# BarisYazici/deep-rl-grasping

Measured on NVIDIA H100. Metric: SAC grad-steps/sec (batch 256, 64x64 depth), higher is better.
Workload: dtype bf16x3 (fp32-faithful split, f32 accumulate)

## Files before the change

### deep-rl-grasping_b200/csrc/engine_v2.cu

```cuda
#include <cuda_bf16.h>

#include <algorithm>
#include <cstdio>
#include <cstdlib>
#include <cstring>

#include "sac_internal.cuh"

namespace b2g {
namespace {

struct Gather2Args {
  GatherArgs g;
  uint16_t* s1[2][3];
  uint16_t* fp[3][3];
  int KF;
};

__device__ __forceinline__ void split3(float y, uint16_t& p0, uint16_t& p1, uint16_t& p2) {
  const __nv_bfloat16 h0 = __float2bfloat16_rn(y);
  const float r1 = y - __bfloat162float(h0);
  const __nv_bfloat16 h1 = __float2bfloat16_rn(r1);
  const float r2 = r1 - __bfloat162float(h1);
  p0 = __bfloat16_as_ushort(h0); p1 = __bfloat16_as_ushort(h1); p2 = __bfloat16_as_ushort(__float2bfloat16_rn(r2));
}

template <int Ci>
__device__ __forceinline__ void s2d_half_block(const Gather2Args& a, const unsigned char* __restrict__ src, int it, int which, size_t b) {
  constexpr int CP = s2d_channels(Ci);
  const GatherArgs& g = a.g;
  const int npx = g.H * g.W * Ci;
  const int h = it & 1, X = (it >> 1) & 15, Y = it >> 5;
  const double clip_obs = g.normc[1];
  const bool norm_obs = g.normc[3] != 0.0;
  const float scale = g.scale;
#pragma unroll
  for (int rr = 0; rr < 2; ++rr) {
    const int e0 = ((4 * Y + 2 * h + rr) * g.W + 4 * X) * Ci;
    float y[4 * Ci];
#pragma unroll
    for (int q = 0; q < Ci; ++q) {
      const int e = e0 + 4 * q;
      const float4 v = frame_load4(src, g.fmt, npx, Ci, e);
      float t[4] = {v.x, v.y, v.z, v.w};
      if (norm_obs) {
        const double2 m0 = *reinterpret_cast<const double2*>(g.mean + e), m1 = *reinterpret_cast<const double2*>(g.mean + e + 2);
        const double2 i0 = *reinterpret_cast<const double2*>(g.var + e), i1 = *reinterpret_cast<const double2*>(g.var + e + 2);
        t[0] = (float)fmin(fmax(((double)t[0] - m0.x) * i0.x, -clip_obs), clip_obs);
        t[1] = (float)fmin(fmax(((double)t[1] - m0.y) * i0.y, -clip_obs), clip_obs);
        t[2] = (float)fmin(fmax(((double)t[2] - m1.x) * i1.x, -clip_obs), clip_obs);
        t[3] = (float)fmin(fmax(((double)t[3] - m1.y) * i1.y, -clip_obs), clip_obs);
      }
#pragma unroll
      for (int j = 0; j < 4; ++j) y[4 * q + j] = t[j];
    }
    uint32_t p[3][2 * CP];
#pragma unroll
    for (int k = 0; k < 4 * CP; k += 2) {
      uint16_t q[3][2];
#pragma unroll
      for (int u = 0; u < 2; ++u) {
        const int c = (k + u) / CP, ci = (k + u) % CP;
        if (ci < Ci) split3(y[c * Ci + ci] / scale, q[0][u], q[1][u], q[2][u]);
        else q[0][u] = q[1][u] = q[2][u] = 0;
      }
#pragma unroll
      for (int pl = 0; pl < 3; ++pl) p[pl][k / 2] = (uint32_t)q[pl][0] | ((uint32_t)q[pl][1] << 16);
    }
    const size_t o = b * 4096 * CP + (size_t)((Y * 16 + X) * 16 + 4 * (2 * h + rr)) * CP;
#pragma unroll
    for (int pl = 0; pl < 3; ++pl) {
      if constexpr (CP == 1) {
        *reinterpret_cast<uint2*>(a.s1[which][pl] + o) = make_uint2(p[pl][0], p[pl][1]);
      } else {
        uint4* d = reinterpret_cast<uint4*>(a.s1[which][pl] + o);
        d[0] = make_uint4(p[pl][0], p[pl][1], p[pl][2], p[pl][3]);
        d[1] = make_uint4(p[pl][4], p[pl][5], p[pl][6], p[pl][7]);
      }
    }
  }
}

template <int Ci>
__global__ void __launch_bounds__(512) gather2_kernel(Gather2Args a) {
  const GatherArgs& g = a.g;
  const int b = blockIdx.x, which = blockIdx.y, tid = threadIdx.x;
  const int HW = g.H * g.W, npx = HW * Ci;
  const int Ec = npx + 4;
  long long slot = b;
  if (g.indices) slot = g.indices[b];
  else if (g.rng_counters) {
    slot = philox_slot(g.seed, (unsigned long long)g.rng_counters[4], b, (unsigned long long)g.rng_counters[5]);
    if (g.ring_cap > 0) slot = ring_slot(g.rng_counters[6], (int)slot, g.ring_cap);
    if (g.indices_out && which == 0 && tid == 0) g.indices_out[b] = (int)slot;
  }
  const unsigned char* __restrict__ src =
      g.obs_frame ? g.frames + (size_t)(which ? g.next_frame : g.obs_frame)[slot] * g.frame_bytes
                  : reinterpret_cast<const unsigned char*>((which ? g.next_obs : g.obs) + (size_t)slot * Ec);
  const double clip_obs = g.normc[1];
  const bool norm_obs = g.normc[3] != 0.0;
  const float scale = g.scale;
  for (int it = tid; it < 512; it += blockDim.x) s2d_half_block<Ci>(a, src, it, which, b);
  if (tid == 0 && g.feat_col >= 0) {
    float yy = frame_elem(src, g.fmt, npx, Ci, npx);
    if (norm_obs) yy = (float)fmin(fmax(((double)yy - g.mean[npx]) * g.var[npx], -clip_obs), clip_obs);
    yy = yy / scale;
    uint16_t p0, p1, p2;
    split3(yy, p0, p1, p2);
    const size_t fo = (size_t)b * g.FS + g.feat_col, po = (size_t)b * a.KF + g.feat_col;
    if (which) { g.F_t[fo] = yy; a.fp[2][0][po] = p0; a.fp[2][1][po] = p1; a.fp[2][2][po] = p2; }
    else {
      g.F_pi[fo] = yy; g.F_v[fo] = yy;
      a.fp[0][0][po] = p0; a.fp[0][1][po] = p1; a.fp[0][2][po] = p2;
      a.fp[1][0][po] = p0; a.fp[1][1][po] = p1; a.fp[1][2][po] = p2;
    }
  }
  if (which == 0 && g.act) {
    const int feat_dim = g.act_col;
    if (tid < g.n_act) {
      const float av = g.act[slot * g.n_act + tid];
      g.F_v[(size_t)b * g.FS + feat_dim + tid] = av;
      uint16_t p0, p1, p2;
      split3(av, p0, p1, p2);
      const size_t po = (size_t)b * a.KF + feat_dim + tid;
      a.fp[1][0][po] = p0; a.fp[1][1][po] = p1; a.fp[1][2][po] = p2;
    }
    if (tid == 32) {
      float r = g.rew[slot];
      if (g.normc[4] != 0.0) r = (float)fmin(fmax((double)r * g.normc[0], -g.normc[2]), g.normc[2]);
      g.rew_out[b] = r;
      g.done_out[b] = g.done[slot];
    }
  }
}

struct Plane2Job {
  const float* src;
  uint16_t* dst[3];
  int R, N, np;
  int transpose;
  int ld, off0;
  int k1_ci;
  int tile_start;
};

constexpr int P2_SUB = 4;
__global__ void __launch_bounds__(256) planes2_kernel(const Plane2Job* __restrict__ jobs, const int* __restrict__ cta_job, int cta0) {
  __shared__ float tile[P2_SUB][64][33];
  const int cta = cta0 + blockIdx.x;
  const Plane2Job job = jobs[cta_job[cta]];
  const int t = cta - job.tile_start;
  const int strips_n = (job.N + 32 * P2_SUB - 1) / (32 * P2_SUB);
  const int r0 = (t / strips_n) * 64, nb = (t % strips_n) * 32 * P2_SUB;
  const int tid = threadIdx.x;
  const bool vec_ok = (job.N & 3) == 0;
  float4 v[P2_SUB][2];
#pragma unroll
  for (int q = 0; q < P2_SUB; ++q)
#pragma unroll
    for (int j = 0; j < 2; ++j) {
      const int i = tid + 256 * j, r = r0 + (i >> 3), n = nb + 32 * q + 4 * (i & 7);
      v[q][j] = make_float4(0.f, 0.f, 0.f, 0.f);
      if (r < job.R && n < job.N) {
        const float* sp = job.src + (size_t)r * job.N + n;
        if (vec_ok && n + 3 < job.N) v[q][j] = *reinterpret_cast<const float4*>(sp);
        else { v[q][j].x = sp[0]; if (n + 1 < job.N) v[q][j].y = sp[1]; if (n + 2 < job.N) v[q][j].z = sp[2]; if (n + 3 < job.N) v[q][j].w = sp[3]; }
      }
    }
#pragma unroll
  for (int q = 0; q < P2_SUB; ++q)
#pragma unroll
    for (int j = 0; j < 2; ++j) {
      const int i = tid + 256 * j, rr = i >> 3, c4 = i & 7, r = r0 + rr, n = nb + 32 * q + 4 * c4;
      if (job.transpose) {
        tile[q][rr][4 * c4] = v[q][j].x; tile[q][rr][4 * c4 + 1] = v[q][j].y; tile[q][rr][4 * c4 + 2] = v[q][j].z; tile[q][rr][4 * c4 + 3] = v[q][j].w;
      } else if (r < job.R && n < job.N) {
        const float x[4] = {v[q][j].x, v[q][j].y, v[q][j].z, v[q][j].w};
        uint16_t p[3][4];
#pragma unroll
        for (int u = 0; u < 4; ++u) split3(x[u], p[0][u], p[1][u], p[2][u]);
#pragma unroll
        for (int k = 0; k < 3; ++k) {
          if (k == job.np) break;
          uint16_t* d = job.dst[k] + (size_t)r * job.ld + job.off0 + n;
          if (n + 3 < job.N && (((size_t)r * job.ld + job.off0 + n) & 3) == 0)
            *reinterpret_cast<uint2*>(d) = make_uint2((uint32_t)p[k][0] | ((uint32_t)p[k][1] << 16), (uint32_t)p[k][2] | ((uint32_t)p[k][3] << 16));
          else
            for (int u = 0; u < 4; ++u) if (n + u < job.N) d[u] = p[k][u];
        }
      }
    }
  if (!job.transpose) return;
  __syncthreads();
  const int nn = tid >> 3, g8 = tid & 7, rb = r0 + 8 * g8;
#pragma unroll
  for (int q = 0; q < P2_SUB; ++q) {
    const int n = nb + 32 * q + nn;
    if (n < job.N && rb < job.R) {
      uint16_t p[3][8];
#pragma unroll
      for (int u = 0; u < 8; ++u) split3(tile[q][8 * g8 + u][nn], p[0][u], p[1][u], p[2][u]);
      const size_t o = (size_t)(n + job.off0) * job.ld + rb;
#pragma unroll
      for (int k = 0; k < 3; ++k) {
        if (k == job.np) break;
        uint16_t* d = job.dst[k] + o;
        if (job.k1_ci) {
          for (int u = 0; u < 8; ++u) if (rb + u < job.R) d[conv1_krow(rb + u, job.k1_ci) - rb] = p[k][u];
        } else if (rb + 7 < job.R && (o & 7) == 0)
          *reinterpret_cast<uint4*>(d) = make_uint4((uint32_t)p[k][0] | ((uint32_t)p[k][1] << 16), (uint32_t)p[k][2] | ((uint32_t)p[k][3] << 16),
                                                    (uint32_t)p[k][4] | ((uint32_t)p[k][5] << 16), (uint32_t)p[k][6] | ((uint32_t)p[k][7] << 16));
        else
          for (int u = 0; u < 8; ++u) if (rb + u < job.R) d[u] = p[k][u];
      }
    }
  }
}

int add_maps(V2State& v, uint16_t* const* planes, int np, int rank, std::initializer_list<uint64_t> dims, std::initializer_list<uint64_t> strides_b,
             std::initializer_list<uint32_t> box, std::initializer_list<uint32_t> estr = {}, bool allow_whole = true, int swizzle = 128) {
  uint64_t d[5] = {1, 1, 1, 1, 1}, s[5] = {0, 0, 0, 0, 0};
  uint32_t bx[5] = {1, 1, 1, 1, 1}, es[5] = {1, 1, 1, 1, 1};
  int i = 0; for (auto x : dims) d[i++] = x;
  i = 0; for (auto x : strides_b) s[i++] = x;
  i = 0; for (auto x : box) bx[i++] = x;
  i = 0; for (auto x : estr) es[i++] = x;
  if (rank >= 5 || np < 1) return -1;
  size_t rows = 1;
  for (int k = 1; k < rank; ++k) rows *= (bx[k] + es[k] - 1) / es[k];
  const size_t box_bytes = rows * bx[0] * 2;
  const bool whole = allow_whole && np > 1 && box_bytes % 1024 == 0;
  const long long pitch = np > 1 ? (long long)((const char*)planes[1] - (const char*)planes[0]) : 16;
  for (int p = 2; p < np; ++p)
    if ((const char*)planes[p] - (const char*)planes[p - 1] != pitch) return -1;
  if (pitch <= 0 || pitch % 16) return -1;
  d[rank] = (uint64_t)np; s[rank - 1] = (uint64_t)pitch; bx[rank] = whole ? (uint32_t)np : 1u; es[rank] = 1;
  CUtensorMap m;
  if (cg_encode_map(&m, planes[0], rank + 1, d, s, bx, es, swizzle) != 0) return -1;
  v.maps.push_back(m);
  v.map_whole.push_back(whole ? 1 : 0);
  v.map_box_bytes.push_back((int)box_bytes);
  return (int)v.maps.size() - 1;
}

const V2State* g_mk_state = nullptr;
CgLoad mk_load(int map, int rank, int smem_off) {
  CgLoad L;
  memset(&L, 0, sizeof(L));
  L.map = map; L.rank = rank + 1; L.smem_off = smem_off;
  L.plane_box = g_mk_state->map_whole[map];
  L.box_bytes = g_mk_state->map_box_bytes[map];
  return L;
}

CgProblem kmajor(int planes, int n_tile, int chunks, int n2, int a_box_rows) {
  CgProblem P;
  memset(&P, 0, sizeof(P));
  P.tiles_m = P.tiles_n = P.splits = 1;
  P.chunks = chunks; P.n2 = n2;
  P.planes = planes;
  P.a_off = 0; P.a_pstride = 128 * 128;
  P.b_off = planes * P.a_pstride; P.b_pstride = n_tile * 128;
  P.tx_bytes = planes * (a_box_rows * 128 + n_tile * 128);
  P.mn_major = 0; P.ksteps = 4; P.a_kstep = P.b_kstep = 32; P.a_kstep2 = 64;
  P.a_desc = P.b_desc = cg_desc_bits(128, false, 0); P.a_moff = 64 * 128;
  P.umma_n = n_tile;
  P.nprod = planes == 3 ? 6 : (planes == 2 ? 3 : 1);
  P.d0 = 1 << 20; P.d1 = 1;
  P.grp_stride = 32; P.f_grp = 32; P.bias_grp = 32;
  P.scale = 1.f;
  return P;
}

CgProblem mnmajor(int planes, int kr, int a_atoms, int b_atoms, int chunks) {
  CgProblem P;
  memset(&P, 0, sizeof(P));
  P.tiles_m = P.tiles_n = P.splits = 1;
  P.chunks = chunks; P.n2 = chunks > 0 ? chunks : 1;
  P.planes = planes;
  const int atom = kr * 128;
  P.a_off = 0; P.a_pstride = atom;
  P.b_off = 2 * planes * atom; P.b_pstride = b_atoms * atom;
  P.tx_bytes = planes * (a_atoms + b_atoms) * atom;
  P.mn_major = 1; P.ksteps = kr / 16; P.a_kstep = P.b_kstep = 2048; P.a_kstep2 = 4096;
  P.a_lbo = planes * atom; P.b_lbo = atom;
  P.a_desc = cg_desc_bits(128, true, P.a_lbo); P.b_desc = cg_desc_bits(128, true, P.b_lbo); P.a_moff = P.a_lbo;
  P.umma_n = 64 * b_atoms;
  P.nprod = planes == 3 ? 6 : (planes == 2 ? 3 : 1);
  P.d0 = 1 << 20; P.d1 = 1;
  P.grp_stride = 32; P.f_grp = 32; P.bias_grp = 32;
  P.scale = 1.f;
  P.epi = CG_EPI_WGRAD; P.rows_tile = 128;
  return P;
}

int push_group(b2g_sac* h, std::vector<CgGroup>& list, CgGroup& g, const char* name) {
  g.name = name;
  if (cg_finalize(g, cg_smem_limit()) != 0) return b2g_fail(B2G_EINVAL, std::string("engine v2: stage ring of group ") + name + " does not fit shared memory");
  for (int i = 0; i < g.n; ++i) {
    const CgProblem& P = g.host[i];
    if (P.planes * P.umma_n > 256) return b2g_fail(B2G_EINVAL, std::string("engine v2: planes x tile width exceeds one accumulator buffer (group ") + name + ")");
    if (!cg_shape_supported(P.umma_n, P.nprod, P.mn_major != 0, P.ksteps))
      return b2g_fail(B2G_EINVAL, std::string("engine v2: no cg_kernel instance for the tile shape of a problem in group ") + name);
    if (P.tm_sub > 1 && !cg_epi_handoff(P.epi))
      return b2g_fail(B2G_EINVAL, std::string("engine v2: a banded problem must have an ACT or DGRAD epilogue (group ") + name + ")");
    g.flops += 2.0 * P.tiles_m * 128.0 * P.tiles_n * P.umma_n * P.chunks * 64.0;
  }
  list.push_back(g);
  return 0;
}

struct Wire { int cons, ci, prod, pi, dep_rows, dep_rows_tile, by_chunk; };
int fuse_groups(b2g_sac* h, const std::vector<const CgGroup*>& parts, const std::vector<Wire>& wires, const char* name, std::vector<CgGroup>& out, int& n_ctr) {
  CgGroup f;
  std::vector<int> first(parts.size());
  for (size_t gi = 0; gi < parts.size(); ++gi) {
    first[gi] = f.n;
    for (int i = 0; i < parts[gi]->n; ++i) {
      if (f.n >= CG_MAX_PROBLEMS) return b2g_fail(B2G_EINVAL, std::string("engine v2: too many problems in fused launch ") + name);
      f.host[f.n++] = parts[gi]->host[i];
    }
  }
  std::vector<int> ctr_of(f.n, -1);
  for (const Wire& w : wires) {
    const int pi = first[w.prod] + w.pi, qi = first[w.cons] + w.ci;
    CgProblem& Pp = f.host[pi];
    CgProblem& Pc = f.host[qi];
    if (!cg_epi_handoff(Pp.epi))
      return b2g_fail(B2G_EINVAL, std::string("engine v2: a wired producer must have an ACT or DGRAD epilogue (fused launch ") + name + ")");
    if (Pc.dep_ctr && ctr_of[pi] < 0) {
      ctr_of[pi] = (int)(intptr_t)Pc.dep_ctr - 1;
      Pc.dep_expect += Pp.ws ? Pp.tiles_n : Pp.tiles_n * Pp.splits;
      continue;
    }
    if (Pp.splits > 1 && (Pp.splits - 1) * ((Pp.chunks + Pp.splits - 1) / Pp.splits) >= Pp.chunks)
      return b2g_fail(B2G_EINVAL, std::string("engine v2: a wired split-K producer has an empty split (fused launch ") + name + ")");
    if (ctr_of[pi] < 0) { ctr_of[pi] = n_ctr; n_ctr += Pp.tiles_m; }
    Pc.dep_rows = w.dep_rows; Pc.dep_rows_tile = w.dep_rows_tile; Pc.dep_tiles = Pp.tiles_m; Pc.dep_by_chunk = w.by_chunk;
    Pc.dep_expect = Pp.ws ? Pp.tiles_n : Pp.tiles_n * Pp.splits;
    Pc.dep_ctr = (const int*)(intptr_t)(ctr_of[pi] + 1);
  }
  for (int i = 0; i < f.n; ++i) f.host[i].done_ctr = (int*)(intptr_t)(ctr_of[i] + 1);
  return push_group(h, out, f, name);
}

void bind_counters(std::vector<CgGroup>& groups, int* base) {
  for (CgGroup& g : groups)
    for (int i = 0; i < g.n; ++i) {
      CgProblem& P = g.host[i];
      const intptr_t d = (intptr_t)P.done_ctr, c = (intptr_t)P.dep_ctr;
      P.done_ctr = d ? base + (d - 1) : nullptr;
      P.dep_ctr = c ? base + (c - 1) : nullptr;
    }
}

int check_split(const char* var, int chunks, int splits) {
  auto empty = [chunks](int s) { return (s - 1) * ((chunks + s - 1) / s) >= chunks; };
  if (!empty(splits)) return 0;
  std::string ok;
  for (int s = 1; s <= chunks; ++s)
    if (!empty(s)) ok += (ok.empty() ? "" : ", ") + std::to_string(s);
  return b2g_fail(B2G_EINVAL, std::string(var) + "=" + std::to_string(splits) + " leaves a K-split of " + std::to_string(chunks) +
                                  " chunks empty; use one of " + ok);
}

}

int v2_alloc(b2g_sac* h) {
  V2State& v = h->v2;
  const int B = h->B, Cp = s2d_channels(h->Cimg), K1 = 64 * Cp, KF = v.KF;
  const size_t n1 = (size_t)B * 225 * 32, n2 = (size_t)B * 36 * 64, n3 = (size_t)B * 1024, ns = (size_t)B * 4096 * Cp, nf = (size_t)B * KF;
  uint16_t *bH1, *bH2, *bH3, *bF, *bS;
  if (int rc = dev_alloc(h->allocs, h->stream, &bH1, 9 * n1)) return rc;
  if (int rc = dev_alloc(h->allocs, h->stream, &bH2, 9 * n2)) return rc;
  if (int rc = dev_alloc(h->allocs, h->stream, &bH3, 9 * n3)) return rc;
  if (int rc = dev_alloc(h->allocs, h->stream, &bF, 9 * nf)) return rc;
  if (int rc = dev_alloc(h->allocs, h->stream, &bS, 6 * ns)) return rc;
  for (int n = 0; n < 3; ++n)
    for (int p = 0; p < 3; ++p) {
      v.H1[n][p] = bH1 + (n * 3 + p) * n1; v.H2[n][p] = bH2 + (n * 3 + p) * n2; v.H3[n][p] = bH3 + (n * 3 + p) * n3;
      v.F[n][p] = bF + (n * 3 + p) * nf;
    }
  for (int w = 0; w < 2; ++w) for (int p = 0; p < 3; ++p) v.S[w][p] = bS + (w * 3 + p) * ns;
  if (int rc = dev_alloc(h->allocs, h->stream, &v.z0v, (size_t)B * 3 * h->H)) return rc;
  auto palloc = [&](uint16_t** arr, int np, size_t count) -> int {
    const size_t pitch = (count + 63) / 64 * 64;
    uint16_t* base = nullptr;
    if (int rc = dev_alloc(h->allocs, h->stream, &base, pitch * np)) return rc;
    for (int p = 0; p < np; ++p) arr[p] = base + p * pitch;
    return 0;
  };
  if (int rc = palloc(v.dz0pi, 2, (size_t)B * h->H)) return rc;
  if (int rc = palloc(v.dz0v, 2, (size_t)B * 3 * h->H)) return rc;
  if (int rc = palloc(v.dZ1, 2, (size_t)B * 225 * 64)) return rc;
  for (int n = 0; n < 2; ++n) {
    if (int rc = palloc(v.dZ4[n], 2, (size_t)B * 512)) return rc;
    if (int rc = palloc(v.dZ3[n], 2, n3)) return rc;
    if (int rc = palloc(v.dZ2[n], 2, n2)) return rc;
    if (int rc = palloc(v.W2n[n], 2, 512 * 64)) return rc;
    if (int rc = palloc(v.W3n[n], 2, 576 * 64)) return rc;
    if (int rc = palloc(v.Wfn[n], 2, 1024 * 512)) return rc;
    if (int rc = palloc(v.K0n[n], 2, (size_t)KF * (n == 1 ? 3 : 1) * h->H)) return rc;
  }
  if (int rc = palloc(v.W1T[0], 3, (size_t)64 * K1)) return rc;
  if (int rc = palloc(v.W1T[1], 3, (size_t)32 * K1)) return rc;
  for (int n = 0; n < 3; ++n) {
    if (int rc = palloc(v.W2T[n], 3, 64 * 512)) return rc;
    if (int rc = palloc(v.W3T[n], 3, 64 * 576)) return rc;
    if (int rc = palloc(v.WfT[n], 3, 512 * 1024)) return rc;
    if (int rc = palloc(v.K0T[n], 3, (size_t)(n == 1 ? 3 : 1) * h->H * KF)) return rc;
  }
  return 0;
}

int v2_create(b2g_sac* h) {
  V2State& v = h->v2;
  g_mk_state = &v;
  const int B = h->B, Ci = h->Cimg, Cp = s2d_channels(Ci), K1 = 64 * Cp, KF = v.KF, FS = h->FS, H = h->H;
  const size_t n1 = (size_t)B * 225 * 32;
  const char* nets[3] = {"model/pi", "model/values_fn", "target/values_fn"};
  std::vector<Plane2Job> jobs;
  int start = 0;
  auto add_job = [&](const float* src, int R, int N, uint16_t* const* dst, int np, int transpose, int ld, int off0) {
    Plane2Job j{};
    j.src = src; j.R = R; j.N = N; j.np = np; j.transpose = transpose; j.ld = ld; j.off0 = off0; j.tile_start = start;
    for (int k = 0; k < np; ++k) j.dst[k] = dst[k];
    start += ((R + 63) / 64) * ((N + 32 * P2_SUB - 1) / (32 * P2_SUB));
    jobs.push_back(j);
  };
  add_job(h->p(h->cnn_t("model/pi", 0, "w")), 64 * Ci, 32, v.W1T[0], 3, 1, K1, 0);
  jobs.back().k1_ci = Ci;
  add_job(h->p(h->cnn_t("model/values_fn", 0, "w")), 64 * Ci, 32, v.W1T[0], 3, 1, K1, 32);
  jobs.back().k1_ci = Ci;
  add_job(h->p(h->cnn_t("target/values_fn", 0, "w")), 64 * Ci, 32, v.W1T[1], 3, 1, K1, 0);
  jobs.back().k1_ci = Ci;
  for (int n = 0; n < 3; ++n) {
    add_job(h->p(h->cnn_t(nets[n], 1, "w")), 512, 64, v.W2T[n], 3, 1, 512, 0);
    add_job(h->p(h->cnn_t(nets[n], 2, "w")), 576, 64, v.W3T[n], 3, 1, 576, 0);
    add_job(h->p(h->cnn_t(nets[n], 3, "w")), 1024, 512, v.WfT[n], 3, 1, 1024, 0);
  }
  add_job(h->p("model/pi/fc0/kernel"), h->feat_dim, H, v.K0T[0], 3, 1, KF, 0);
  add_job(h->p("model/values_fn/vf/fc0/kernel"), h->feat_dim, H, v.K0T[1], 3, 1, KF, 0);
  add_job(h->p("model/values_fn/qf1/fc0/kernel"), h->feat_dim + h->A, H, v.K0T[1], 3, 1, KF, H);
  add_job(h->p("model/values_fn/qf2/fc0/kernel"), h->feat_dim + h->A, H, v.K0T[1], 3, 1, KF, 2 * H);
  add_job(h->p("target/values_fn/vf/fc0/kernel"), h->feat_dim, H, v.K0T[2], 3, 1, KF, 0);
  v.plane_ctas_fwd = start;
  for (int n = 0; n < 2; ++n) {
    add_job(h->p(h->cnn_t(nets[n], 1, "w")), 512, 64, v.W2n[n], 2, 0, 64, 0);
    add_job(h->p(h->cnn_t(nets[n], 2, "w")), 576, 64, v.W3n[n], 2, 0, 64, 0);
    add_job(h->p(h->cnn_t(nets[n], 3, "w")), 1024, 512, v.Wfn[n], 2, 0, 512, 0);
  }
  add_job(h->p("model/pi/fc0/kernel"), h->feat_dim, H, v.K0n[0], 2, 0, H, 0);
  add_job(h->p("model/values_fn/vf/fc0/kernel"), h->feat_dim, H, v.K0n[1], 2, 0, 3 * H, 0);
  add_job(h->p("model/values_fn/qf1/fc0/kernel"), h->feat_dim + h->A, H, v.K0n[1], 2, 0, 3 * H, H);
  add_job(h->p("model/values_fn/qf2/fc0/kernel"), h->feat_dim + h->A, H, v.K0n[1], 2, 0, 3 * H, 2 * H);
  v.n_plane_jobs = (int)jobs.size();
  v.plane_ctas = start;
  Plane2Job* dj = nullptr;
  if (int rc = dev_alloc(h->allocs, h->stream, &dj, jobs.size())) return rc;
  CK(cudaMemcpyAsync(dj, jobs.data(), jobs.size() * sizeof(Plane2Job), cudaMemcpyHostToDevice, h->stream));
  CK(cudaStreamSynchronize(h->stream));
  v.plane_jobs = dj;
  {
    std::vector<int> cj((size_t)start);
    for (size_t k = 0; k < jobs.size(); ++k)
      for (int t = jobs[k].tile_start; t < (k + 1 < jobs.size() ? jobs[k + 1].tile_start : start); ++t) cj[t] = (int)k;
    if (int rc = upload_table(h->allocs, h->stream, cj, &v.plane_cta_job)) return rc;
  }

  { const char* e = getenv("B2G_SPLIT_FC1"); v.split_fc1 = e ? std::max(1, atoi(e)) : 3; }
  { const char* e = getenv("B2G_SPLIT_FC1_DGRAD"); v.split_fc1_dgrad = e ? std::max(1, atoi(e)) : 1; }
  const int NP = 3;
  const long long h1_net = (long long)3 * n1;
  {
    CgGroup g;
    for (int w = 0; w < 2; ++w) {
      const int N = w == 0 ? 64 : 32;
      const int mA = Cp == 1 ? add_maps(v, v.S[w], NP, 3, {32, 15, (uint64_t)B * 16}, {32, 512}, {32, 16, 8}, {}, true, 64)
                             : add_maps(v, v.S[w], NP, 3, {64, 16, (uint64_t)B * 16}, {128, 2048}, {64, 16, 8});
      const int mB = add_maps(v, v.W1T[w], NP, 2, {(uint64_t)K1, (uint64_t)N}, {(uint64_t)K1 * 2}, {64, (uint32_t)N});
      if (mA < 0 || mB < 0) return b2g_fail(B2G_ECUDA, "engine v2: cuTensorMapEncodeTiled failed (conv1)");
      CgProblem P;
      if (Cp == 1) {
        P = kmajor(NP, N, 1, 1, 128);
        P.a_pstride = 128 * 64; P.a_kstep = 32; P.a_kstep2 = NP * P.a_pstride;
        P.b_off = 2 * P.a_kstep2;
        P.tx_bytes = NP * (2 * 128 * 64 + N * 128);
        P.a_desc = cg_desc_bits(64, false, 0); P.a_moff = 64 * 64;
        P.nloads = 3;
        for (int a = 0; a < 2; ++a) { P.ld[a] = mk_load(mA, 3, a * P.a_kstep2); P.ld[a].c0[2] = a; P.ld[a].d_tm[2] = 8; }
        P.ld[2] = mk_load(mB, 2, P.b_off);
      } else {
        P = kmajor(NP, N, 4, 2, 128);
        P.nloads = 2;
        P.ld[0] = mk_load(mA, 3, 0); P.ld[0].d_tm[2] = 8; P.ld[0].d_c1[2] = 1; P.ld[0].d_c2[1] = 1;
        P.ld[1] = mk_load(mB, 2, P.b_off); P.ld[1].d_c1[0] = 128; P.ld[1].d_c2[0] = 64;
      }
      P.tiles_m = 2 * B;
      P.epi = CG_EPI_ACT; P.rows_tile = 128; P.lim_rows = 2 * B * 128;
      P.d0 = 16; P.d1 = 8; P.o0 = 32; P.o1 = 15 * 32; P.o_tm = 225 * 32;
      P.tm_sub = 2; P.o_sub = 8 * 15 * 32; P.lim_i0 = 15; P.lim_i1 = 15;
      P.n_valid = N; P.out_planes = 3;
      P.grp_stride = (int)h1_net;
      const int net0 = w == 0 ? 0 : 2;
      for (int p = 0; p < 3; ++p) P.out_p[p] = v.H1[net0][p];
      P.bias = h->p(h->cnn_t(nets[net0], 0, "b"));
      P.bias_grp = w == 0 ? (int)(h->p(h->cnn_t("model/values_fn", 0, "b")) - h->p(h->cnn_t("model/pi", 0, "b"))) : 32;
      g.host[g.n++] = P;
    }
    if (int rc = push_group(h, v.fwd, g, "conv1_fwd")) return rc;
  }
  {
    CgGroup g;
    for (int n = 0; n < 3; ++n) {
      const int mA = add_maps(v, v.H1[n], NP, 4, {64, 14, 15, (uint64_t)B}, {64, 15 * 64, 225 * 64}, {64, 12, 12, 3}, {1, 2, 2, 1});
      const int mB = add_maps(v, v.W2T[n], NP, 2, {512, 64}, {1024}, {64, 64});
      if (mA < 0 || mB < 0) return b2g_fail(B2G_ECUDA, "engine v2: cuTensorMapEncodeTiled failed (conv2)");
      CgProblem P = kmajor(NP, 64, 8, 2, 108);
      P.nloads = 2;
      P.ld[0] = mk_load(mA, 4, 0); P.ld[0].d_tm[3] = 3; P.ld[0].d_c1[2] = 1; P.ld[0].d_c2[1] = 2;
      P.ld[1] = mk_load(mB, 2, P.b_off); P.ld[1].d_c1[0] = 128; P.ld[1].d_c2[0] = 64;
      P.tiles_m = (B + 2) / 3;
      P.epi = CG_EPI_ACT; P.rows_tile = 108; P.lim_rows = B * 36;
      P.o_tm = 108 * 64; P.o0 = 64; P.n_valid = 64; P.out_planes = 3;
      for (int p = 0; p < 3; ++p) P.out_p[p] = v.H2[n][p];
      P.bias = h->p(h->cnn_t(nets[n], 1, "b")); P.bias_grp = 32;
      g.host[g.n++] = P;
    }
    if (int rc = push_group(h, v.fwd, g, "conv2_fwd")) return rc;
  }
  {
    CgGroup g;
    for (int n = 0; n < 3; ++n) {
      const int mA = add_maps(v, v.H2[n], NP, 4, {64, 6, 6, (uint64_t)B}, {128, 6 * 128, 36 * 128}, {64, 4, 4, 8});
      const int mB = add_maps(v, v.W3T[n], NP, 2, {576, 64}, {1152}, {64, 64});
      if (mA < 0 || mB < 0) return b2g_fail(B2G_ECUDA, "engine v2: cuTensorMapEncodeTiled failed (conv3)");
      CgProblem P = kmajor(NP, 64, 9, 3, 128);
      P.nloads = 2;
      P.ld[0] = mk_load(mA, 4, 0); P.ld[0].d_tm[3] = 8; P.ld[0].d_c1[2] = 1; P.ld[0].d_c2[1] = 1;
      P.ld[1] = mk_load(mB, 2, P.b_off); P.ld[1].d_c1[0] = 192; P.ld[1].d_c2[0] = 64;
      P.tiles_m = (B + 7) / 8;
      P.epi = CG_EPI_ACT; P.rows_tile = 128; P.lim_rows = B * 16;
      P.o_tm = 128 * 64; P.o0 = 64; P.n_valid = 64; P.out_planes = 3;
      for (int p = 0; p < 3; ++p) P.out_p[p] = v.H3[n][p];
      P.bias = h->p(h->cnn_t(nets[n], 2, "b")); P.bias_grp = 32;
// ... 222 lines not shown
        P.b_off = 2 * P.a_lbo;
        P.tx_bytes = NB * (2 * 64 * 64 + 64 * 128);
        P.a_kstep = 16 * 64; P.a_kstep2 = 2 * P.a_kstep; P.a_desc = cg_desc_bits(64, true, P.a_lbo); P.a_moff = 0;
        P.nloads = 3;
        for (int a = 0; a < 2; ++a) { P.ld[a] = mk_load(mA, 3, a * P.a_lbo); P.ld[a].c0[2] = a; P.ld[a].d_c1[2] = 16; P.ld[a].d_c2[2] = 4; }
        P.tiles_m = 1;
        P.d0 = 4; P.d1 = 4; P.o0 = 32; P.o1 = 8 * 32;
        P.rgrp_rows = 16;
        for (int l = 0; l < 4; ++l) P.rgrp_off[l] = (32 * (l >> 1) + 4 * (l & 1)) * 32;
      } else {
        for (int l = 0; l < 2; ++l) {
          P.ld[l] = mk_load(mA, 3, l * P.a_lbo); P.ld[l].c0[1] = l; P.ld[l].d_tm[2] = 1; P.ld[l].d_c1[2] = 16; P.ld[l].d_c2[2] = 4;
        }
        P.nloads = 3;
        P.tiles_m = 2;
        P.d0 = 4; P.d1 = 4; P.o0 = 32; P.o1 = Ci * 32; P.o_tm = 32 * Ci * 32;
        P.lim_i0 = Ci;
        P.rgrp_rows = 16;
        for (int j = 0; j < 8; ++j) P.rgrp_off[j] = (8 * Ci * (j & 3) + 4 * Ci * (j >> 2)) * 32;
      }
      P.ld[P.nloads - 1] = mk_load(mB, 4, P.b_off); P.ld[P.nloads - 1].d_c1[3] = 1; P.ld[P.nloads - 1].d_c2[2] = 4;
      P.tiles_n = 1;
      P.splits = std::max(1, std::min(P.chunks, std::max(84 / P.tiles_m, (P.chunks + 15) / 16)));
      P.lim_rows = 64 * Cp; P.n_valid = 64;
      P.out_f = h->g(h->cnn_t("model/pi", 0, "w")); P.f_grp = (long long)(h->g(h->cnn_t("model/values_fn", 0, "w")) - h->g(h->cnn_t("model/pi", 0, "w"))); P.atomic = 1;
      g.host[g.n++] = P;
    }
    if (int rc = push_group(h, v.bwd_groups, g, "conv_wgrad")) return rc;
  }
  int n_ctr = 0;
  {
    std::vector<const CgGroup*> parts;
    for (auto& g : v.fwd) parts.push_back(&g);
    std::vector<Wire> w;
    for (int n = 0; n < 3; ++n) {
      w.push_back({1, n, 0, n < 2 ? 0 : 1, 6, 1, 0});
      w.push_back({2, n, 1, n, 8 * 36, 108, 0});
      w.push_back({3, n, 2, n, 128 * 16, 128, 0});
      w.push_back({4, n, 3, n, 128, 128, 0});
    }
    if (int rc = fuse_groups(h, parts, w, "fwd_fused", v.fwd_fused, n_ctr)) return rc;
  }
  {
    std::vector<const CgGroup*> parts;
    for (auto& g : v.bwd_groups) parts.push_back(&g);
    std::vector<Wire> w;
    for (int n = 0; n < 2; ++n) {
      w.push_back({1, 2 * n, 0, n, 128, 128, 0});
      w.push_back({1, 2 * n + 1, 0, n, 64, 128, 1});
      w.push_back({2, 2 * n, 1, 2 * n, 3, 128, 0});
      w.push_back({2, 2 * n + 1, 1, 2 * n, 4, 128, 1});
      w.push_back({3, n, 2, 2 * n, 72, 108, 0});
      w.push_back({4, n, 2, 2 * n, 144, 108, 1});
    }
    w.push_back({4, 2, 3, 0, 1, 8, 1});
    w.push_back({4, 2, 3, 1, 1, 8, 1});
    if (int rc = fuse_groups(h, parts, w, "bwd_fused", v.bwd_fused, n_ctr)) return rc;
    std::vector<const CgGroup*> pa(parts.begin(), parts.begin() + 2), pb(parts.begin() + 2, parts.end());
    std::vector<Wire> wa, wb;
    for (int n = 0; n < 2; ++n) {
      wa.push_back({1, 2 * n, 0, n, 128, 128, 0});
      wa.push_back({1, 2 * n + 1, 0, n, 64, 128, 1});
      wb.push_back({1, n, 0, 2 * n, 72, 108, 0});
      wb.push_back({2, n, 0, 2 * n, 144, 108, 1});
    }
    wb.push_back({2, 2, 1, 0, 1, 8, 1});
    wb.push_back({2, 2, 1, 1, 1, 8, 1});
    if (int rc = fuse_groups(h, pa, wa, "bwd_fused_fc", v.bwd_fused, n_ctr)) return rc;
    if (int rc = fuse_groups(h, pb, wb, "bwd_fused_conv", v.bwd_fused, n_ctr)) return rc;
  }
  if (int rc = dev_alloc(h->allocs, h->stream, &v.dep_ctr, (size_t)n_ctr)) return rc;
  v.n_dep_ctr = n_ctr;
  bind_counters(v.fwd_fused, v.dep_ctr);
  bind_counters(v.bwd_fused, v.dep_ctr);
  if (int rc = dev_alloc(h->allocs, h->stream, &v.d_maps, v.maps.size())) return rc;
  CK(cudaMemcpyAsync(v.d_maps, v.maps.data(), v.maps.size() * sizeof(CUtensorMap), cudaMemcpyHostToDevice, h->stream));
  CK(cudaStreamSynchronize(h->stream));
  return 0;
}

int v2_planes(b2g_sac* h, bool backward, cudaStream_t s) {
  V2State& v = h->v2;
  const int cta0 = backward ? v.plane_ctas_fwd : 0, n = backward ? v.plane_ctas - v.plane_ctas_fwd : v.plane_ctas_fwd;
  planes2_kernel<<<n, 256, 0, s>>>((const Plane2Job*)v.plane_jobs, v.plane_cta_job, cta0);
  return 0;
}

int v2_gather(b2g_sac* h, const GatherArgs& ga, cudaStream_t s) {
  V2State& v = h->v2;
  Gather2Args a{};
  a.g = ga;
  for (int w = 0; w < 2; ++w)
    for (int p = 0; p < 3; ++p) a.s1[w][p] = v.S[w][p];
  for (int n = 0; n < 3; ++n) for (int p = 0; p < 3; ++p) a.fp[n][p] = v.F[n][p];
  a.KF = v.KF;
  const dim3 grid(ga.B, ga.next_obs || ga.next_frame ? 2 : 1);
  switch (h->Cimg) {
    case 1: gather2_kernel<1><<<grid, 512, 0, s>>>(a); break;
    case 2: gather2_kernel<2><<<grid, 512, 0, s>>>(a); break;
    case 3: gather2_kernel<3><<<grid, 512, 0, s>>>(a); break;
    default: gather2_kernel<4><<<grid, 512, 0, s>>>(a); break;
  }
  return 0;
}

extern long long* g_cg_trace;
static long long* s_trace_buf = nullptr;

int v2_launch(b2g_sac* h, const CgGroup& g, cudaStream_t s) {
  const char* tn = getenv("B2G_CG_TRACE");
  cudaStreamCaptureStatus cs0 = cudaStreamCaptureStatusNone;
  if (tn) cudaStreamIsCapturing(s, &cs0);
  if (tn && cs0 == cudaStreamCaptureStatusNone && std::string(tn) == g.name) {
    if (!s_trace_buf) cudaMalloc(&s_trace_buf, 640 * sizeof(long long));
    cudaMemsetAsync(s_trace_buf, 0, 640 * sizeof(long long), s);
    g_cg_trace = s_trace_buf;
    const char* tc = getenv("B2G_CG_TRACE_CTA");
    cudaError_t e = cg_launch(g, h->v2.d_maps, h->num_sms - h->v2.sm_reserve, s, false, h->v2.dbg | ((tc ? atoi(tc) : 0) << 8));
    g_cg_trace = nullptr;
    if (e != cudaSuccess) return b2g_fail(B2G_ECUDA, cudaGetErrorString(e));
    static int shots = 0;
    if (shots++ == 3) {
      long long t[640];
      cudaStreamSynchronize(s);
      cudaMemcpy(t, s_trace_buf, sizeof(t), cudaMemcpyDeviceToHost);
      const long long t0 = t[0];
      fprintf(stderr, "cg trace %s (cycles; per chunk: prod wait_start wait_done issued | mma wait_start full_seen committed)\n", g.name);
      for (int i = 0; i < 64 && t[i * 8 + 2]; ++i)
        fprintf(stderr, "  chunk %2d (p %lld tm %lld): %7lld %7lld %7lld | %7lld %7lld %7lld\n", i, t[i * 8 + 6] / 100000, t[i * 8 + 6] % 100000 / 10, t[i * 8] - t0,
                t[i * 8 + 1] - t0, t[i * 8 + 2] - t0, t[i * 8 + 3] - t0, t[i * 8 + 4] - t0, t[i * 8 + 5] - t0);
      for (int i = 0; i < 16 && t[512 + i * 4 + 1]; ++i)
        fprintf(stderr, "  tile %d (p %lld tm %lld) mma: start %7lld sums out %7lld (%s)\n", i, t[512 + i * 4 + 3] / 100000, t[512 + i * 4 + 3] % 100000 / 10,
                t[512 + i * 4] - t0, t[512 + i * 4 + 1] - t0, t[512 + i * 4 + 2] ? "handed off" : "in place");
      for (int i = 0; i < 16 && t[576 + i * 4 + 2]; ++i)
        fprintf(stderr, "  handoff %d (p %lld tm %lld) epilogue warpgroup: buffer wait %7lld start %7lld end %7lld\n", i, t[576 + i * 4 + 3] / 100000,
                t[576 + i * 4 + 3] % 100000 / 10, t[576 + i * 4] - t0, t[576 + i * 4 + 1] - t0, t[576 + i * 4 + 2] - t0);
    }
    return 0;
  }
  CK(cg_launch(g, h->v2.d_maps, h->num_sms - h->v2.sm_reserve, s, pdl_enabled(), h->v2.dbg));
  return 0;
}

}
```

Baseline: 2567.

## Make gather and plane-split kernels persistent with register double-buffered prefetch

The gather kernel now uses fixed 128-thread CTAs. Each CTA owns one spatial slice and loops over many images, resolving all image source pointers up front into shared memory. It caches the per-pixel normalization mean and variance in shared memory and prefetches the next image(s) into registers while storing the current one. The planes kernel likewise becomes a grid-stride persistent loop with next-strip prefetch and a register cap, and uses a smaller grid for the backward pass. This aims to cut launch and tail overhead and redundant mean/var loads, at the risk of lower parallelism and serialized per-image metadata work in blockIdx.x==0 CTAs.

```diff
diff --git a/deep-rl-grasping_b200/csrc/engine_v2.cu b/deep-rl-grasping_b200/csrc/engine_v2.cu
--- a/deep-rl-grasping_b200/csrc/engine_v2.cu
+++ b/deep-rl-grasping_b200/csrc/engine_v2.cu
@@ -25,31 +25,42 @@
   p0 = __bfloat16_as_ushort(h0); p1 = __bfloat16_as_ushort(h1); p2 = __bfloat16_as_ushort(__float2bfloat16_rn(r2));
 }
 
+constexpr int G2_THREADS = 128;
+template <int Ci> __host__ __device__ constexpr int g2_depth() { return Ci == 1 ? 2 : 1; }
+template <int Ci> __host__ __device__ constexpr int g2_ctas_per_sm() { return Ci >= 3 ? 2 : 4; }
+constexpr size_t g2_smem(int Ci, int max_imgs) { return (size_t)16 * Ci * G2_THREADS * sizeof(double) + (size_t)max_imgs * sizeof(void*); }
+
 template <int Ci>
-__device__ __forceinline__ void s2d_half_block(const Gather2Args& a, const unsigned char* __restrict__ src, int it, int which, size_t b) {
+__device__ __forceinline__ void g2_load(const Gather2Args& a, const unsigned char* __restrict__ src, int it, float4 (&v)[2][Ci]) {
+  const GatherArgs& g = a.g;
+  const int npx = g.H * g.W * Ci;
+  const int h = it & 1, X = (it >> 1) & 15, Y = it >> 5;
+#pragma unroll
+  for (int rr = 0; rr < 2; ++rr)
+#pragma unroll
+    for (int q = 0; q < Ci; ++q) v[rr][q] = frame_load4(src, g.fmt, npx, Ci, ((4 * Y + 2 * h + rr) * g.W + 4 * X) * Ci + 4 * q);
+}
+
+template <int Ci>
+__device__ __forceinline__ void g2_store(const Gather2Args& a, const float4 (&v)[2][Ci], const double* st, int it, int which, size_t b) {
   constexpr int CP = s2d_channels(Ci);
   const GatherArgs& g = a.g;
-  const int npx = g.H * g.W * Ci;
   const int h = it & 1, X = (it >> 1) & 15, Y = it >> 5;
   const double clip_obs = g.normc[1];
   const bool norm_obs = g.normc[3] != 0.0;
   const float scale = g.scale;
 #pragma unroll
   for (int rr = 0; rr < 2; ++rr) {
-    const int e0 = ((4 * Y + 2 * h + rr) * g.W + 4 * X) * Ci;
     float y[4 * Ci];
 #pragma unroll
     for (int q = 0; q < Ci; ++q) {
-      const int e = e0 + 4 * q;
-      const float4 v = frame_load4(src, g.fmt, npx, Ci, e);
-      float t[4] = {v.x, v.y, v.z, v.w};
+      float t[4] = {v[rr][q].x, v[rr][q].y, v[rr][q].z, v[rr][q].w};
       if (norm_obs) {
-        const double2 m0 = *reinterpret_cast<const double2*>(g.mean + e), m1 = *reinterpret_cast<const double2*>(g.mean + e + 2);
-        const double2 i0 = *reinterpret_cast<const double2*>(g.var + e), i1 = *reinterpret_cast<const double2*>(g.var + e + 2);
-        t[0] = (float)fmin(fmax(((double)t[0] - m0.x) * i0.x, -clip_obs), clip_obs);
-        t[1] = (float)fmin(fmax(((double)t[1] - m0.y) * i0.y, -clip_obs), clip_obs);
-        t[2] = (float)fmin(fmax(((double)t[2] - m1.x) * i1.x, -clip_obs), clip_obs);
-        t[3] = (float)fmin(fmax(((double)t[3] - m1.y) * i1.y, -clip_obs), clip_obs);
+#pragma unroll
+        for (int j = 0; j < 4; ++j) {
+          const int k = 4 * Ci * rr + 4 * q + j;
+          t[j] = (float)fmin(fmax(((double)t[j] - st[k * G2_THREADS]) * st[(8 * Ci + k) * G2_THREADS], -clip_obs), clip_obs);
+        }
       }
 #pragma unroll
       for (int j = 0; j < 4; ++j) y[4 * q + j] = t[j];
@@ -82,55 +93,98 @@
 }
 
 template <int Ci>
-__global__ void __launch_bounds__(512) gather2_kernel(Gather2Args a) {
+__global__ void __launch_bounds__(G2_THREADS, Ci >= 3 ? 4 : 6) gather2_kernel(Gather2Args a, int n_img) {
+  extern __shared__ double g2_sm[];
   const GatherArgs& g = a.g;
-  const int b = blockIdx.x, which = blockIdx.y, tid = threadIdx.x;
+  const int tid = threadIdx.x, it = blockIdx.x * G2_THREADS + tid, G = gridDim.y;
+  const int n_mine = (n_img - (int)blockIdx.y + G - 1) / G;
   const int HW = g.H * g.W, npx = HW * Ci;
   const int Ec = npx + 4;
-  long long slot = b;
-  if (g.indices) slot = g.indices[b];
-  else if (g.rng_counters) {
-    slot = philox_slot(g.seed, (unsigned long long)g.rng_counters[4], b, (unsigned long long)g.rng_counters[5]);
-    if (g.ring_cap > 0) slot = ring_slot(g.rng_counters[6], (int)slot, g.ring_cap);
-    if (g.indices_out && which == 0 && tid == 0) g.indices_out[b] = (int)slot;
-  }
-  const unsigned char* __restrict__ src =
-      g.obs_frame ? g.frames + (size_t)(which ? g.next_frame : g.obs_frame)[slot] * g.frame_bytes
-                  : reinterpret_cast<const unsigned char*>((which ? g.next_obs : g.obs) + (size_t)slot * Ec);
   const double clip_obs = g.normc[1];
   const bool norm_obs = g.normc[3] != 0.0;
   const float scale = g.scale;
-  for (int it = tid; it < 512; it += blockDim.x) s2d_half_block<Ci>(a, src, it, which, b);
-  if (tid == 0 && g.feat_col >= 0) {
-    float yy = frame_elem(src, g.fmt, npx, Ci, npx);
-    if (norm_obs) yy = (float)fmin(fmax(((double)yy - g.mean[npx]) * g.var[npx], -clip_obs), clip_obs);
-    yy = yy / scale;
-    uint16_t p0, p1, p2;
-    split3(yy, p0, p1, p2);
-    const size_t fo = (size_t)b * g.FS + g.feat_col, po = (size_t)b * a.KF + g.feat_col;
-    if (which) { g.F_t[fo] = yy; a.fp[2][0][po] = p0; a.fp[2][1][po] = p1; a.fp[2][2][po] = p2; }
-    else {
-      g.F_pi[fo] = yy; g.F_v[fo] = yy;
-      a.fp[0][0][po] = p0; a.fp[0][1][po] = p1; a.fp[0][2][po] = p2;
-      a.fp[1][0][po] = p0; a.fp[1][1][po] = p1; a.fp[1][2][po] = p2;
-    }
-  }
-  if (which == 0 && g.act) {
-    const int feat_dim = g.act_col;
-    if (tid < g.n_act) {
-      const float av = g.act[slot * g.n_act + tid];
-      g.F_v[(size_t)b * g.FS + feat_dim + tid] = av;
+  const unsigned char** srcs = reinterpret_cast<const unsigned char**>(g2_sm + 16 * Ci * G2_THREADS);
+  for (int k = tid; k < n_mine; k += G2_THREADS) {
+    const int i = blockIdx.y + k * G, which = i >= g.B, b = i - which * g.B;
+    long long slot = b;
+    if (g.indices) slot = g.indices[b];
+    else if (g.rng_counters) {
+      slot = philox_slot(g.seed, (unsigned long long)g.rng_counters[4], b, (unsigned long long)g.rng_counters[5]);
+      if (g.ring_cap > 0) slot = ring_slot(g.rng_counters[6], (int)slot, g.ring_cap);
+      if (g.indices_out && which == 0 && blockIdx.x == 0) g.indices_out[b] = (int)slot;
+    }
+    const unsigned char* __restrict__ src =
+        g.obs_frame ? g.frames + (size_t)(which ? g.next_frame : g.obs_frame)[slot] * g.frame_bytes
+                    : reinterpret_cast<const unsigned char*>((which ? g.next_obs : g.obs) + (size_t)slot * Ec);
+    srcs[k] = src;
+    if (blockIdx.x != 0) continue;
+    if (g.feat_col >= 0) {
+      float yy = frame_elem(src, g.fmt, npx, Ci, npx);
+      if (norm_obs) yy = (float)fmin(fmax(((double)yy - g.mean[npx]) * g.var[npx], -clip_obs), clip_obs);
+      yy = yy / scale;
       uint16_t p0, p1, p2;
-      split3(av, p0, p1, p2);
-      const size_t po = (size_t)b * a.KF + feat_dim + tid;
-      a.fp[1][0][po] = p0; a.fp[1][1][po] = p1; a.fp[1][2][po] = p2;
-    }
-    if (tid == 32) {
+      split3(yy, p0, p1, p2);
+      const size_t fo = (size_t)b * g.FS + g.feat_col, po = (size_t)b * a.KF + g.feat_col;
+      if (which) { g.F_t[fo] = yy; a.fp[2][0][po] = p0; a.fp[2][1][po] = p1; a.fp[2][2][po] = p2; }
+      else {
+        g.F_pi[fo] = yy; g.F_v[fo] = yy;
+        a.fp[0][0][po] = p0; a.fp[0][1][po] = p1; a.fp[0][2][po] = p2;
+        a.fp[1][0][po] = p0; a.fp[1][1][po] = p1; a.fp[1][2][po] = p2;
+      }
+    }
+    if (which == 0 && g.act) {
+      const int feat_dim = g.act_col;
+      for (int j = 0; j < g.n_act; ++j) {
+        const float av = g.act[slot * g.n_act + j];
+        g.F_v[(size_t)b * g.FS + feat_dim + j] = av;
+        uint16_t p0, p1, p2;
+        split3(av, p0, p1, p2);
+        const size_t po = (size_t)b * a.KF + feat_dim + j;
+        a.fp[1][0][po] = p0; a.fp[1][1][po] = p1; a.fp[1][2][po] = p2;
+      }
       float r = g.rew[slot];
       if (g.normc[4] != 0.0) r = (float)fmin(fmax((double)r * g.normc[0], -g.normc[2]), g.normc[2]);
       g.rew_out[b] = r;
       g.done_out[b] = g.done[slot];
     }
+  }
+  __syncthreads();
+  constexpr int D = g2_depth<Ci>();
+  float4 cur[D][2][Ci], nxt[D][2][Ci];
+#pragma unroll
+  for (int d = 0; d < D; ++d)
+    if (d < n_mine) g2_load<Ci>(a, srcs[d], it, cur[d]);
+  double* st = g2_sm + tid;
+  if (norm_obs) {
+    const int h = it & 1, X = (it >> 1) & 15, Y = it >> 5;
+#pragma unroll
+    for (int rr = 0; rr < 2; ++rr)
+#pragma unroll
+      for (int q = 0; q < Ci; ++q) {
+        const int e = ((4 * Y + 2 * h + rr) * g.W + 4 * X) * Ci + 4 * q, k = 4 * Ci * rr + 4 * q;
+        const double2 m0 = *reinterpret_cast<const double2*>(g.mean + e), m1 = *reinterpret_cast<const double2*>(g.mean + e + 2);
+        const double2 i0 = *reinterpret_cast<const double2*>(g.var + e), i1 = *reinterpret_cast<const double2*>(g.var + e + 2);
+        st[k * G2_THREADS] = m0.x; st[(k + 1) * G2_THREADS] = m0.y; st[(k + 2) * G2_THREADS] = m1.x; st[(k + 3) * G2_THREADS] = m1.y;
+        st[(8 * Ci + k) * G2_THREADS] = i0.x; st[(8 * Ci + k + 1) * G2_THREADS] = i0.y;
+        st[(8 * Ci + k + 2) * G2_THREADS] = i1.x; st[(8 * Ci + k + 3) * G2_THREADS] = i1.y;
+      }
+  }
+  for (int k0 = 0; k0 < n_mine; k0 += D) {
+#pragma unroll
+    for (int d = 0; d < D; ++d)
+      if (k0 + D + d < n_mine) g2_load<Ci>(a, srcs[k0 + D + d], it, nxt[d]);
+#pragma unroll
+    for (int d = 0; d < D; ++d)
+      if (k0 + d < n_mine) {
+        const int i = blockIdx.y + (k0 + d) * G, which = i >= g.B;
+        g2_store<Ci>(a, cur[d], st, it, which, (size_t)(i - which * g.B));
+      }
+#pragma unroll
+    for (int d = 0; d < D; ++d)
+#pragma unroll
+      for (int rr = 0; rr < 2; ++rr)
+#pragma unroll
+        for (int q = 0; q < Ci; ++q) cur[d][rr][q] = nxt[d][rr][q];
   }
 }
 
@@ -145,21 +199,22 @@
 };
 
 constexpr int P2_SUB = 4;
-__global__ void __launch_bounds__(256) planes2_kernel(const Plane2Job* __restrict__ jobs, const int* __restrict__ cta_job, int cta0) {
-  __shared__ float tile[P2_SUB][64][33];
-  const int cta = cta0 + blockIdx.x;
-  const Plane2Job job = jobs[cta_job[cta]];
-  const int t = cta - job.tile_start;
-  const int strips_n = (job.N + 32 * P2_SUB - 1) / (32 * P2_SUB);
-  const int r0 = (t / strips_n) * 64, nb = (t % strips_n) * 32 * P2_SUB;
-  const int tid = threadIdx.x;
+struct P2Strip { Plane2Job job; int r0, nb; };
+__device__ __forceinline__ P2Strip p2_strip(const Plane2Job* __restrict__ jobs, const int* __restrict__ cta_job, int cta) {
+  P2Strip s;
+  s.job = jobs[cta_job[cta]];
+  const int t = cta - s.job.tile_start, strips_n = (s.job.N + 32 * P2_SUB - 1) / (32 * P2_SUB);
+  s.r0 = (t / strips_n) * 64; s.nb = (t % strips_n) * 32 * P2_SUB;
+  return s;
+}
+__device__ __forceinline__ void p2_load(const P2Strip& s, int tid, float4 (&v)[P2_SUB][2]) {
+  const Plane2Job& job = s.job;
   const bool vec_ok = (job.N & 3) == 0;
-  float4 v[P2_SUB][2];
 #pragma unroll
   for (int q = 0; q < P2_SUB; ++q)
 #pragma unroll
     for (int j = 0; j < 2; ++j) {
-      const int i = tid + 256 * j, r = r0 + (i >> 3), n = nb + 32 * q + 4 * (i & 7);
+      const int i = tid + 256 * j, r = s.r0 + (i >> 3), n = s.nb + 32 * q + 4 * (i & 7);
       v[q][j] = make_float4(0.f, 0.f, 0.f, 0.f);
       if (r < job.R && n < job.N) {
         const float* sp = job.src + (size_t)r * job.N + n;
@@ -167,6 +222,10 @@
         else { v[q][j].x = sp[0]; if (n + 1 < job.N) v[q][j].y = sp[1]; if (n + 2 < job.N) v[q][j].z = sp[2]; if (n + 3 < job.N) v[q][j].w = sp[3]; }
       }
     }
+}
+__device__ __forceinline__ void p2_store(const P2Strip& s, int tid, const float4 (&v)[P2_SUB][2], float (*tile)[64][33]) {
+  const Plane2Job& job = s.job;
+  const int r0 = s.r0, nb = s.nb;
 #pragma unroll
   for (int q = 0; q < P2_SUB; ++q)
 #pragma unroll
@@ -214,6 +273,28 @@
           for (int u = 0; u < 8; ++u) if (rb + u < job.R) d[u] = p[k][u];
       }
     }
+  }
+  __syncthreads();
+}
+__global__ void __maxnreg__(96) planes2_kernel(const Plane2Job* __restrict__ jobs, const int* __restrict__ cta_job, int cta0, int n_strips) {
+  __shared__ float tile[P2_SUB][64][33];
+  const int tid = threadIdx.x;
+  int t = blockIdx.x;
+  if (t >= n_strips) return;
+  P2Strip cur = p2_strip(jobs, cta_job, cta0 + t);
+  float4 v[P2_SUB][2];
+  p2_load(cur, tid, v);
+  for (; t < n_strips; t += gridDim.x) {
+    const int tn = t + gridDim.x;
+    P2Strip nxt = cur;
+    float4 vn[P2_SUB][2];
+    if (tn < n_strips) { nxt = p2_strip(jobs, cta_job, cta0 + tn); p2_load(nxt, tid, vn); }
+    p2_store(cur, tid, v, tile);
+    cur = nxt;
+#pragma unroll
+    for (int q = 0; q < P2_SUB; ++q)
+#pragma unroll
+      for (int j = 0; j < 2; ++j) v[q][j] = vn[q][j];
   }
 }
 
@@ -362,6 +443,21 @@
     if (!empty(s)) ok += (ok.empty() ? "" : ", ") + std::to_string(s);
   return b2g_fail(B2G_EINVAL, std::string(var) + "=" + std::to_string(splits) + " leaves a K-split of " + std::to_string(chunks) +
                                   " chunks empty; use one of " + ok);
+}
+
+template <int Ci>
+int g2_groups(int n_img, int num_sms) { return std::max(1, std::min(n_img, num_sms * g2_ctas_per_sm<Ci>() / 4)); }
+
+template <int Ci>
+cudaError_t gather2_setup(int B, int num_sms) {
+  const int G = g2_groups<Ci>(2 * B, num_sms);
+  return cudaFuncSetAttribute(gather2_kernel<Ci>, cudaFuncAttributeMaxDynamicSharedMemorySize, (int)g2_smem(Ci, (2 * B + G - 1) / G));
+}
+
+template <int Ci>
+void gather2_launch(const Gather2Args& a, int n_img, int num_sms, cudaStream_t s) {
+  const int G = g2_groups<Ci>(n_img, num_sms);
+  gather2_kernel<Ci><<<dim3(4, G), G2_THREADS, g2_smem(Ci, (n_img + G - 1) / G), s>>>(a, n_img);
 }
 
 }
@@ -461,6 +557,11 @@
   CK(cudaMemcpyAsync(dj, jobs.data(), jobs.size() * sizeof(Plane2Job), cudaMemcpyHostToDevice, h->stream));
   CK(cudaStreamSynchronize(h->stream));
   v.plane_jobs = dj;
+  {
+    cudaError_t e = Ci == 1 ? gather2_setup<1>(B, h->num_sms) : Ci == 2 ? gather2_setup<2>(B, h->num_sms)
+                  : Ci == 3 ? gather2_setup<3>(B, h->num_sms) : gather2_setup<4>(B, h->num_sms);
+    if (e != cudaSuccess) return b2g_fail(B2G_ECUDA, std::string("engine v2: gather shared memory: ") + cudaGetErrorString(e));
+  }
   {
     std::vector<int> cj((size_t)start);
     for (size_t k = 0; k < jobs.size(); ++k)
@@ -849,7 +950,8 @@
 int v2_planes(b2g_sac* h, bool backward, cudaStream_t s) {
   V2State& v = h->v2;
   const int cta0 = backward ? v.plane_ctas_fwd : 0, n = backward ? v.plane_ctas - v.plane_ctas_fwd : v.plane_ctas_fwd;
-  planes2_kernel<<<n, 256, 0, s>>>((const Plane2Job*)v.plane_jobs, v.plane_cta_job, cta0);
+  const int grid = std::max(1, std::min(n, backward ? h->num_sms / 4 : h->num_sms));
+  planes2_kernel<<<grid, 256, 0, s>>>((const Plane2Job*)v.plane_jobs, v.plane_cta_job, cta0, n);
   return 0;
 }
 
@@ -861,12 +963,12 @@
     for (int p = 0; p < 3; ++p) a.s1[w][p] = v.S[w][p];
   for (int n = 0; n < 3; ++n) for (int p = 0; p < 3; ++p) a.fp[n][p] = v.F[n][p];
   a.KF = v.KF;
-  const dim3 grid(ga.B, ga.next_obs || ga.next_frame ? 2 : 1);
+  const int n_img = ga.B * (ga.next_obs || ga.next_frame ? 2 : 1);
   switch (h->Cimg) {
-    case 1: gather2_kernel<1><<<grid, 512, 0, s>>>(a); break;
-    case 2: gather2_kernel<2><<<grid, 512, 0, s>>>(a); break;
-    case 3: gather2_kernel<3><<<grid, 512, 0, s>>>(a); break;
-    default: gather2_kernel<4><<<grid, 512, 0, s>>>(a); break;
+    case 1: gather2_launch<1>(a, n_img, h->num_sms, s); break;
+    case 2: gather2_launch<2>(a, n_img, h->num_sms, s); break;
+    case 3: gather2_launch<3>(a, n_img, h->num_sms, s); break;
+    default: gather2_launch<4>(a, n_img, h->num_sms, s); break;
   }
   return 0;
 }
```

Result: no change. 2546, median of 6 (-0.8%).
